# kcat/openal-soft

Hardware: NVIDIA H100
Metric: voice-samples/s mixed (HRTF, bsinc24, 1024-frame updates) (higher is better)
Workload: dtype f32

## Files before the change

openal-soft_b200/csrc/b200mix.cu:

```cuda
#include "../../include/b200mix.h"

#include <algorithm>
#include <cmath>
#include <cstdio>
#include <cstdlib>
#include <cstring>
#include <new>
#include <string>
#include <vector>

#include <cuda_runtime.h>

#include <dlfcn.h>

#include "mixer_kernels.cuh"
#include "effect_kernels.cuh"
#include "shard_kernels.cuh"
#include "panmix_tc.cuh"
#include "param_kernels.hpp"
#include "efx_kernels.hpp"
#include "resampler_tables.hpp"
#include "hrtf_store.hpp"
#include "adpcm.hpp"

// ... 145 lines not shown
    uint32_t num_order{0};
    bool order_dirty{true};

    char *h_src{nullptr}, *d_src{nullptr}; uint32_t src_cap{0};
    cudaEvent_t src_done{nullptr}; bool src_busy{false};
    bool dev_filters{false};
    bool panmix_tc{false};
    bool mix_gather_only{false};

    struct Shard {
        uint32_t rank{0}, world{1}; int transport{0};
        char *own{nullptr}; size_t bytes{0};
        char *peer[kShardMaxWorld]{};
        size_t off_real{0}, off_wet{0}, real_floats{0}, wet_src_floats{0};
        uint32_t owned_max{0};
        uint32_t epoch{0};
        uint32_t *d_counters{nullptr};
        uint32_t *h_status{nullptr};
        cudaEvent_t ev[4]{};
        bool ev_wet{false}, ev_real{false};
        void *nccl_lib{nullptr}; void *comm{nullptr};
        int (*reduce)(const void*, void*, size_t, int, int, int, void*, cudaStream_t){nullptr};
        int (*allreduce)(const void*, void*, size_t, int, int, void*, cudaStream_t){nullptr};
        int (*comm_destroy)(void*){nullptr};
    } shard;

    uint32_t ir_pad{0};
    uint32_t voice_hi{0};
    int mix_variant{0}; int mix_groups{2}; int mix_gs{64}; int mix_cdr{0};
    uint32_t reverb_seq{0};
    size_t mix_smem{0}; int mix_blocks_per_sm{1};
    uint32_t *d_claim{nullptr};
    int fir_blocks_per_sm{0};
};

namespace {

#define CUDA_TRY(dev, expr) do { cudaError_t e_ = (expr); if(e_ != cudaSuccess) {            \
    (dev)->error = std::string(#expr) + ": " + cudaGetErrorString(e_); return B200MIX_ERR_CUDA; } } while(0)

template<typename T>
int dev_alloc(b200mix_device *d, T *&p, size_t count, bool zero = true)
{
    p = nullptr;
    if(count == 0) return B200MIX_OK;
    CUDA_TRY(d, cudaMalloc(reinterpret_cast<void**>(&p), count*sizeof(T)));
    if(zero) CUDA_TRY(d, cudaMemsetAsync(p, 0, count*sizeof(T), d->stream));
    return B200MIX_OK;
}

using MixKernel = void(*)(const MixParams);

struct Variant { MixKernel fn; int gs, groups, cdr; size_t smem; };

template<int GS, int GROUPS, int CDR>
Variant make_variant()
{
    return Variant{k_mix_voices<GS, GROUPS, CDR>, GS, GROUPS, CDR, sizeof(GroupSmem<CDR>)*GROUPS};
}

Variant get_variant(int idx)
{
    return idx == 0 ? make_variant<64, 2, 4>() : make_variant<64, 2, 0>();
}

struct FirVariant { MixKernel fn; size_t smem; };
// ... 144 lines not shown
        if(int rc = dev_alloc(d, d->d_dry_cur, size_t(dd.max_voices)*std::max(dd.dry_channels, 1u))) return rc;
        if(int rc = dev_alloc(d, d->d_dry_tgt, size_t(dd.max_voices)*std::max(dd.dry_channels, 1u))) return rc;
        if(dd.num_sends && dd.wet_channels)
        {
            const size_t per = size_t(dd.num_sends)*dd.wet_channels;
            if(int rc = dev_alloc(d, d->d_send_cur, dd.max_voices*per)) return rc;
            if(int rc = dev_alloc(d, d->d_send_tgt, dd.max_voices*per)) return rc;
        }
        if(int rc = dev_alloc(d, d->d_order, dd.max_voices)) return rc;
        d->h_active.assign(dd.max_voices, 0);
        d->h_cost.assign(dd.max_voices, 0);
        d->h_hrtf.assign(dd.max_voices, 0);

        const bool hrtfDev = dd.ir_size > 0;
        d->mix_variant = (!hrtfDev && dd.dry_channels <= 4) ? 0 : 1;
        const Variant var = get_variant(d->mix_variant);
        d->mix_gs = var.gs; d->mix_groups = var.groups; d->mix_cdr = var.cdr; d->mix_smem = var.smem;
        CUDA_TRY(d, cudaFuncSetAttribute(var.fn, cudaFuncAttributeMaxDynamicSharedMemorySize, int(var.smem)));
        int perSm = 0;
        CUDA_TRY(d, cudaOccupancyMaxActiveBlocksPerMultiprocessor(&perSm, var.fn, var.gs*var.groups, var.smem));
        d->mix_blocks_per_sm = std::max(perSm, 1);
        if(var.cdr == 0)
        {
            if(int rc = dev_alloc(d, d->d_xscratch, size_t(dd.max_voices)*kLine)) return rc;
            if(int rc = dev_alloc(d, d->d_sendinfo, dd.max_voices)) return rc;
            if(int rc = dev_alloc(d, d->d_claim, 2)) return rc;
        }
        if(hrtfDev)
        {
            const FirVariant fir = get_fir(dd.ir_size);
            CUDA_TRY(d, cudaFuncSetAttribute(fir.fn, cudaFuncAttributeMaxDynamicSharedMemorySize, int(fir.smem)));
            CUDA_TRY(d, cudaOccupancyMaxActiveBlocksPerMultiprocessor(&perSm, fir.fn, kFirGS*kFirGroups, fir.smem));
            d->fir_blocks_per_sm = std::max(std::min(perSm, kFirCtasPerSm), 1);
        }

        d->dry_alloc_ch = std::max<uint32_t>(std::max(dd.dry_channels, 1u), uint32_t(var.cdr));
        if(int rc = dev_alloc(d, d->d_dry, size_t(d->dry_alloc_ch)*kLine)) return rc;
        {
            const size_t realFloats = size_t(std::max(dd.real_channels, 1u))*kLine;
            static_assert(sizeof(VoiceResult) == 16 && sizeof(b200mix_voice_result) == 16, "result layout");
            const size_t blockBytes = realFloats*sizeof(float) + size_t(dd.max_voices)*sizeof(VoiceResult);
            char *blk = nullptr;
            if(int rc = dev_alloc(d, blk, blockBytes)) return rc;
            d->d_outblock = blk;
            d->d_results = reinterpret_cast<VoiceResult*>(blk + realFloats*sizeof(float));
            CUDA_TRY(d, cudaMallocHost(reinterpret_cast<void**>(&d->h_outblock), blockBytes));
            d->h_real = reinterpret_cast<float*>(d->h_outblock);
            d->h_results = reinterpret_cast<b200mix_voice_result*>(d->h_outblock + realFloats*sizeof(float));
            d->out_real_bytes = realFloats*sizeof(float);
            if(dd.post_process == B200MIX_POST_NONE) d->d_real = d->d_dry;
            else d->d_real = reinterpret_cast<float*>(blk);
        }
        if(dd.max_slots && dd.wet_channels)
            if(int rc = dev_alloc(d, d->d_wet, size_t(dd.max_slots)*dd.wet_channels*kLine)) return rc;
        d->partial_floats = hrtfDev ? size_t(d->num_sms)*d->fir_blocks_per_sm*(2*kAccumLen)
            : size_t(d->num_sms)*d->mix_blocks_per_sm*size_t(var.cdr)*kLine;
        if(int rc = dev_alloc(d, d->d_partial, std::max<size_t>((hrtfDev ? 1 : 2)*d->partial_floats, 4))) return rc;
        if(int rc = dev_alloc(d, d->d_accum_sum, 2*kAccumLen)) return rc;
        if(int rc = dev_alloc(d, d->d_carry[0], 2*kHrirLen)) return rc;
        if(int rc = dev_alloc(d, d->d_carry[1], 2*kHrirLen)) return rc;
        if(int rc = dev_alloc(d, d->d_temp, size_t(std::max(dd.dry_channels, 1u))*kLine)) return rc;
        if(int rc = dev_alloc(d, d->d_temp2, size_t(std::max(dd.dry_channels, 1u))*kLine)) return rc;
        if(dd.max_slots && dd.wet_channels && dd.num_sends)
        {
            d->h_slots.assign(dd.max_slots, SlotRec{});
            d->slot_allocs.assign(dd.max_slots, {});
// ... 30 lines not shown
        }
        if(int rc = ensure_stage(d, std::min(dd.max_voices, 4096u))) return rc;
        CUDA_TRY(d, cudaStreamSynchronize(d->stream));
        return B200MIX_OK;
    };
    int rc;
    try { rc = run(); }
    catch(const std::exception &e) { d->error = e.what(); rc = B200MIX_ERR_NOMEM; }
    if(rc != B200MIX_OK) return fail(rc);
    *out = d;
    return B200MIX_OK;
}

void b200mix_destroy(b200mix_device *d)
{
    if(!d) return;
    if(d->stream) cudaStreamSynchronize(d->stream);
    shard_release(d);
    for(auto &b : d->h_buffers) if(b.data) cudaFree(const_cast<void*>(b.data));
    for(int i = 0;i < 3;++i) cudaFree(d->d_bsinc[i]);
    for(int i = 0;i < 2;++i) cudaFree(d->d_cubic[i]);
    cudaFree(d->d_voices); cudaFree(d->d_buffers); cudaFree(d->d_hrtf_tgt); cudaFree(d->d_hrtf_old);
    cudaFree(d->d_dry_cur); cudaFree(d->d_dry_tgt); cudaFree(d->d_send_cur); cudaFree(d->d_send_tgt);
    cudaFree(d->d_outblock); cudaFreeHost(d->h_outblock); cudaFree(d->d_order);
    cudaFree(d->d_dry); cudaFree(d->d_wet); cudaFree(d->d_partial); cudaFree(d->d_accum_sum);
    cudaFree(d->d_carry[0]); cudaFree(d->d_carry[1]);
    cudaFree(d->d_dec_coef); cudaFree(d->d_dec_hfscale); cudaFree(d->d_dec_state);
    cudaFree(d->d_temp); cudaFree(d->d_temp2);
    cudaFree(d->d_amb_hf); cudaFree(d->d_amb_lf); cudaFree(d->d_amb_state);
    cudaFree(d->d_uhj_state); cudaFree(d->d_uhj_scratch);
    cudaFree(d->d_uhj_fir_state); cudaFree(d->d_uhj_fir_coef); cudaFree(d->d_bs2b); cudaFree(d->d_stab_state);
    for(auto &v : d->slot_allocs) for(void *p : v) cudaFree(p);
    cudaFree(d->d_slots); cudaFree(d->d_xscratch); cudaFree(d->d_sendinfo); cudaFree(d->d_claim);
    cudaFree(d->d_filt); cudaFree(d->d_fupd); cudaFree(d->d_fscratch);
    cudaFree(d->d_dline); cudaFree(d->d_order2); cudaFree(d->d_qhdr); cudaFree(d->d_queue);
    cudaFree(d->d_outbuf); if(d->h_outbuf) cudaFreeHost(d->h_outbuf);
    cudaFree(d->d_limiter); cudaFree(d->d_limiter_delay);
    cudaFree(d->d_dc_delay); cudaFree(d->d_dc_gain); cudaFree(d->d_dc_buf);
    cudaFree(d->d_st_fields); cudaFree(d->d_st_elevs); cudaFree(d->d_st_coeffs); cudaFree(d->d_st_delays);
    cudaFree(d->d_dry_entries); cudaFree(d->d_dry_slot_start); cudaFree(d->d_dry_partial);
    cudaFree(d->d_dry_geff); cudaFree(d->d_send_geff); cudaFree(d->d_send_partial);
    cudaFree(d->d_dry_gramp); cudaFree(d->d_send_gramp);
    if(d->h_fupd) cudaFreeHost(d->h_fupd);
    if(d->fstage_done) cudaEventDestroy(d->fstage_done);
    cudaFree(d->d_slot_start); cudaFree(d->d_entries); cudaFree(d->d_twiddle); cudaFree(d->d_cubic_filter);
    cudaFree(d->d_efx_views);
    cudaFreeHost(d->h_arena); cudaFree(d->d_arena);
    if(d->h_src) cudaFreeHost(d->h_src);
    cudaFree(d->d_src);
    if(d->src_done) cudaEventDestroy(d->src_done);
    if(d->stage_done) cudaEventDestroy(d->stage_done);
    if(d->ev_mix0) cudaEventDestroy(d->ev_mix0);
    if(d->ev_mix1) cudaEventDestroy(d->ev_mix1);
    for(cudaEvent_t e : d->ev_stage) if(e) cudaEventDestroy(e);
    if(d->stream) cudaStreamDestroy(d->stream);
    delete d;
}

int b200mix_set_hrtf_decoder(b200mix_device *d, uint32_t channels, uint32_t ir_size,
    const float *coeffs, const float *hf_scale, const float *splitter_coeff)
{
    if(!d || channels != d->desc.dry_channels || ir_size > B200MIX_HRIR_LENGTH || !coeffs
        || !hf_scale || !splitter_coeff || d->desc.post_process != B200MIX_POST_HRTF)
    { if(d) d->error = "set_hrtf_decoder: bad arguments"; return B200MIX_ERR_INVALID; }
    CUDA_TRY(d, cudaSetDevice(d->cuda_dev));
    cudaFree(d->d_dec_coef); cudaFree(d->d_dec_hfscale); cudaFree(d->d_dec_state);
// ... 1115 lines not shown
        if(d->num_order2)
        {
            CUDA_TRY(d, cudaMemcpyAsync(d->d_order2, d->h_order2.data(), d->num_order2*sizeof(uint32_t),
                cudaMemcpyHostToDevice, d->stream));
            CUDA_TRY(d, cudaStreamSynchronize(d->stream));
        }
        d->order2_dirty = false;
    }
    const Variant var = get_variant(d->mix_variant);
    const bool hrtfDev = dd.ir_size > 0;
    const uint32_t nv = std::max(d->voice_hi, 1u);
    const uint32_t maxBlocks = uint32_t(d->num_sms*d->mix_blocks_per_sm);
    const uint32_t blocks = std::max(1u, std::min(maxBlocks, (d->num_order + var.groups - 1)/var.groups));

    MixParams P{};
    P.voices = d->d_voices; P.buffers = d->d_buffers;
    P.hrtf_tgt = d->d_hrtf_tgt; P.hrtf_old = d->d_hrtf_old;
    P.dry_cur = d->d_dry_cur; P.dry_tgt = d->d_dry_tgt;
    P.send_cur = d->d_send_cur; P.send_tgt = d->d_send_tgt;
    P.dry = d->d_dry; P.wet = d->d_wet; P.partial = d->d_partial;
    P.results = want_results ? d->d_results : nullptr;
    for(int i = 0;i < 3;++i) P.bsinc_tab[i] = d->d_bsinc[i];
    for(int i = 0;i < 2;++i) P.cubic_tab[i] = d->d_cubic[i];
    P.max_voices = nv; P.frames = frames; P.ir = dd.ir_size; P.ir_pad = d->ir_pad;
    P.cd = dd.dry_channels; P.cw = dd.wet_channels; P.num_sends = dd.num_sends;
    P.max_buffers = dd.max_buffers;
    P.order = d->d_order; P.num_order = d->num_order;
    P.xscratch = d->d_xscratch; P.sendinfo = d->d_sendinfo;
    P.filt = d->d_filt; P.filt_paths = 1u + dd.num_sends;
    P.qhdr = d->d_qhdr; P.queue = d->d_queue;
    P.gather_only = d->mix_gather_only ? 1u : 0u;
    P.claim = d->d_claim;
    P.dline = d->d_dline;
    stage_mark(d, 1);
    if(d->profile) cudaEventRecord(d->ev_mix0, d->stream);
    var.fn<<<blocks, var.gs*var.groups, var.smem, d->stream>>>(P);
    ++d->launches;
    CUDA_TRY(d, cudaGetLastError());

    stage_mark(d, 2);
    size_t rows2 = 0;
    if(d->d_filt && d->num_order2)
    {
        FilterRunParams FP{};
        FP.filt = d->d_filt; FP.filt_paths = 1u + dd.num_sends; FP.sendinfo = d->d_sendinfo;
        FP.direct_order = d->d_order2; FP.num_direct = d->num_order2;
        FP.xscratch = d->d_xscratch; FP.dline = d->d_dline; FP.frames = frames;
        k_filters<<<(d->num_order2 + 31u)/32u, 32, 0, d->stream>>>(FP);
        ++d->launches;
        if(var.cdr > 0)
        {
            const uint32_t blocks2 = std::max(1u, std::min(maxBlocks, (d->num_order2 + var.groups - 1)/var.groups));
            rows2 = blocks2;
            MixParams P2 = P;
            P2.pass = 1u;
            P2.order = d->d_order2; P2.num_order = d->num_order2;
            P2.partial = d->d_partial + d->partial_floats;
            P2.results = nullptr;
            var.fn<<<blocks2, var.gs*var.groups, var.smem, d->stream>>>(P2);
            ++d->launches;
        }
        CUDA_TRY(d, cudaGetLastError());
    }
    uint32_t firBlocks = 0;
    if(hrtfDev)
    {
        const FirVariant fir = get_fir(dd.ir_size);
        firBlocks = std::max(1u, std::min(uint32_t(d->num_sms*d->fir_blocks_per_sm),
            (d->num_order + kFirGroups - 1)/kFirGroups));
        fir.fn<<<firBlocks, kFirGS*kFirGroups, fir.smem, d->stream>>>(P);
        ++d->launches;
        CUDA_TRY(d, cudaGetLastError());
    }
    if(d->profile) { cudaEventRecord(d->ev_mix1, d->stream); d->ev_valid = true; }

    stage_mark(d, 3);
    if(hrtfDev)
    {
        const uint32_t len = 2*kAccumLen;
        k_reduce_rows<<<(len/4 + kReduceCols - 1)/kReduceCols, 1024, 0, d->stream>>>(d->d_partial, firBlocks, len,
            d->d_accum_sum, 0);
        ++d->launches;
    }
    if(var.cdr > 0)
    {
        const uint32_t len = uint32_t(var.cdr)*kLine;
        k_reduce_rows<<<(len/4 + kReduceCols - 1)/kReduceCols, 1024, 0, d->stream>>>(d->d_partial, blocks, len, d->d_dry, 1);
        ++d->launches;
        if(rows2)
        {
            k_reduce_rows<<<(len/4 + kReduceCols - 1)/kReduceCols, 1024, 0, d->stream>>>(d->d_partial + d->partial_floats,
                uint32_t(rows2), len, d->d_dry, 1);
            ++d->launches;
        }
    }
    CUDA_TRY(d, cudaGetLastError());

    stage_mark(d, 4);
    if(var.cdr == 0 && d->d_dry_entries)
    {
        if(d->dry_entries_dirty)
        {
            d->h_dry_entries.clear();
            for(uint32_t v = 0;v < d->voice_hi;++v)
                if(d->h_active[v] && !d->h_hrtf[v]) d->h_dry_entries.push_back(SendEntry{v, 0u});
            d->num_dry_entries = uint32_t(d->h_dry_entries.size());
// ... 439 lines not shown
static int render_launch(b200mix_device *d, uint32_t frames, bool want_results)
{
    if(d->mid_render) { d->error = "render: a render_begin is pending"; return B200MIX_ERR_INVALID; }
    const bool sharded = d->shard.transport != 0;
    if(sharded) ++d->shard.epoch;
    if(int rc = render_phase_a(d, frames, want_results, sharded)) return rc;
    if(sharded) if(int rc = shard_wet_exchange(d)) return rc;
    if(int rc = render_phase_b(d, frames)) return rc;
    if(sharded) if(int rc = shard_real_reduce(d)) return rc;
    return render_output_stage(d, frames);
}

static int render_collect(b200mix_device *d, uint32_t frames, float *const *real_out,
    b200mix_voice_result *results)
{
    const b200mix_device_desc &dd = d->desc;
    const uint32_t nv = std::max(d->voice_hi, 1u);
    const bool contiguous = d->d_real == reinterpret_cast<float*>(d->d_outblock);
    if(real_out && results && contiguous)
        CUDA_TRY(d, cudaMemcpyAsync(d->h_outblock, d->d_outblock, d->out_real_bytes + size_t(nv)*sizeof(VoiceResult),
            cudaMemcpyDeviceToHost, d->stream));
    else
    {
        if(real_out)
            CUDA_TRY(d, cudaMemcpyAsync(d->h_real, d->d_real, size_t(dd.real_channels)*kLine*sizeof(float),
                cudaMemcpyDeviceToHost, d->stream));
        if(results)
            CUDA_TRY(d, cudaMemcpyAsync(d->h_results, d->d_results, size_t(nv)*sizeof(VoiceResult),
                cudaMemcpyDeviceToHost, d->stream));
    }
    if(d->shard.transport == 1)
        CUDA_TRY(d, cudaMemcpyAsync(d->shard.h_status, d->shard.own + offsetof(ShardCtl, status),
            sizeof(uint32_t), cudaMemcpyDeviceToHost, d->stream));
    CUDA_TRY(d, cudaStreamSynchronize(d->stream));
    d->stage_busy = false;
    if(d->shard.transport == 1 && *d->shard.h_status)
    { d->error = "render: a peer of the sharded device set did not answer in time"; return B200MIX_ERR_CUDA; }
    if(real_out)
        for(uint32_t c = 0;c < dd.real_channels;++c)
            if(real_out[c]) std::memcpy(real_out[c], d->h_real + size_t(c)*kLine, frames*sizeof(float));
    if(results)
    {
        std::memcpy(results, d->h_results, size_t(nv)*sizeof(b200mix_voice_result));
        for(uint32_t v = nv;v < dd.max_voices;++v)
            results[v] = b200mix_voice_result{0, 0u, B200MIX_VF_STOPPED, 0u};
    }
    return B200MIX_OK;
}

int b200mix_render(b200mix_device *d, uint32_t frames, float *const *real_out,
    b200mix_voice_result *results)
{
    if(!d) return B200MIX_ERR_INVALID;
    if(int rc = render_launch(d, frames, results != nullptr)) return rc;
    return render_collect(d, frames, real_out, results);
}

int b200mix_set_uhj_encoder(b200mix_device *d, uint32_t filter_length, uint32_t *delay)
{
    if(!d) return B200MIX_ERR_INVALID;
    const b200mix_device_desc &dd = d->desc;
    if(d->mid_render || (dd.post_process != B200MIX_POST_UHJ && dd.post_process != B200MIX_POST_TSME)
        || dd.dry_channels < 3
        || (filter_length != 0 && filter_length != 256 && filter_length != 512))
    { d->error = "set_uhj_encoder: needs a UHJ device and a length of 0, 256 or 512"; return B200MIX_ERR_INVALID; }
    CUDA_TRY(d, cudaStreamSynchronize(d->stream));
    CUDA_TRY(d, cudaMemset(d->d_uhj_state, 0, 64*sizeof(float)));
    if(filter_length)
// ... 460 lines not shown
```

openal-soft_b200/csrc/mixer_kernels.cuh:

```cuda
#pragma once
#include <cstdint>
#include <cuda_runtime.h>

#include "voice_structs.hpp"
#include "async_ptx.cuh"

namespace b200mix {

constexpr int kLine = 1024;
constexpr int kHrirLen = 128;
constexpr int kHist = 64;
constexpr int kEdge = 24;
constexpr int kPad = 48;
constexpr int kResBuf = kLine + 256 + kPad;
constexpr int kSrcSizeMax = kResBuf - kEdge;
constexpr int kAccumLen = kLine + kHrirLen;
constexpr float kSilence = 0.00001f;
constexpr float kEps = 1.1920929e-07f;

constexpr uint32_t kVfStatic = 1u<<2, kVfLooping = 1u<<3, kVfHrtf = 1u<<4;
constexpr uint32_t kVfFading = 1u<<8, kVfHaveBuffer = 1u<<9, kVfCoefDirty = 1u<<10;
constexpr uint32_t kUpNoBuffer = 1u<<11;
constexpr uint32_t kVfChannelMask = 0xffu<<16;

struct alignas(16) BufferRec {
    const void *data;
    uint32_t frames, type, channels, pad;
};

struct alignas(16) VoiceRec {
    uint32_t state;
    uint32_t flags;
    uint32_t buffer, resampler;
// ... 10 lines not shown

struct alignas(16) FilterRec {
    float cur[2][5]; float tgt[2][5];
    float z[2][2];
    int32_t counter[2];
    uint32_t active;
    uint32_t pad[5];
};
static_assert(sizeof(FilterRec) == 128, "FilterRec layout");

struct MixParams {
    VoiceRec *voices; const BufferRec *buffers;
    float2 *hrtf_tgt; float2 *hrtf_old;
    float *dry_cur; float *dry_tgt;
    float *send_cur; float *send_tgt;
    float *dry;
    float *wet;
    float *partial;
    VoiceResult *results;
    const float *bsinc_tab[3];
    const float *cubic_tab[2];
    uint32_t max_voices, frames, ir, ir_pad, cd, cw, num_sends, max_buffers;
    float *xscratch;
    uint32_t *sendinfo;
    const uint32_t *order;
    uint32_t num_order;
    FilterRec *filt;
    uint32_t filt_paths;
    uint32_t pass;
    const float *dline;
    uint4 *qhdr; const uint32_t *queue;
    uint32_t gather_only;
    uint32_t *claim;
};

constexpr uint32_t kMaxQueue = 32, kNoLoop = 0xffffffffu;

constexpr uint32_t kSiSend = 1u, kSiPlaying = 2u, kSiDeferred = 4u, kSiDirty = 8u, kSiDry = 16u,
    kSiHrtf = 32u;

__device__ __forceinline__ void group_sync(int id, int count)
{
    if(id == 1) asm volatile("bar.sync 1, %0;" :: "r"(count) : "memory");
    else asm volatile("bar.sync 2, %0;" :: "r"(count) : "memory");
}

__device__ __forceinline__ void prefetch_l2(const void *p)
{ asm volatile("prefetch.global.L2 [%0];" :: "l"(p)); }

__device__ __forceinline__ uint32_t sample_bytes(uint32_t type)
{ return type == 1u ? 2u : ((type == 0u || type >= 5u) ? 1u : (type == 4u ? 8u : 4u)); }

__device__ __forceinline__ void prefetch_span(const char *base, size_t bytes, size_t off,
    size_t len, int t, int gs)
{
    if(off >= bytes) return;
    if(off + len > bytes) len = bytes - off;
    const size_t first = off & ~size_t(127);
    for(size_t a = first + size_t(t)*128u;a < off + len;a += size_t(gs)*128u)
        prefetch_l2(base + a);
}

__device__ __forceinline__ float load_sample(const BufferRec &b, size_t idx)
{
    switch(b.type)
    {
// ... 88 lines not shown
            k = k < A.count ? k : A.count-1u;
            uint32_t q;
            if(!A.looping) q = min(A.uintPos + k, A.lastFrame);
            else if(k < A.firstRun) q = A.q0 + k;
            else if(A.simpleWrap) q = A.loopStart + (k - A.firstRun);
            else q = A.loopStart + (k - A.firstRun)%A.loopSize;
            raw[u] = ld_raw(src + size_t(q)*A.channels);
        }
        #pragma unroll
        for(int u = 0;u < 8;++u)
        {
            const uint32_t k = k0 + uint32_t(u)*GS;
            if(k < A.count) A.dst[k] = A.pastEnd ? 0.0f : to_float(raw[u]);
        }
    }
}

template<int CDR>
struct alignas(16) GroupSmem {
    static constexpr int kTabStride = kPad + 2;
    float win[kResBuf + 8 + 24];
    alignas(8) float tabF[32*kTabStride];
    alignas(8) float tabD[32*kTabStride];
    float x[CDR > 0 ? kLine : 1];
    float newGain[32];
    uint64_t tmaBar;
    uint32_t claimed;
};

template<int GS, int OPT, int FP>
struct alignas(16) FirSmem {
    static constexpr int kLLen = FP + OPT*GS;
    static constexpr int kOLen = FP + kHist + FP + 32;
    float2 lLR[kLLen];
    float2 oLR[kOLen];
    float x[kHist + kLine];
    float2 coefT[kHrirLen], coefO[kHrirLen];
};

__device__ __forceinline__ float2 fma2_rn(float2 a, float2 b, float2 c)
{ return make_float2(__fmaf_rn(a.x, b.x, c.x), __fmaf_rn(a.y, b.y, c.y)); }

template<int OPT, int FP>
__device__ __forceinline__ void fir_pass(float2 (&acc)[OPT], const float2 *__restrict__ in,
    const float2 *__restrict__ coef, int irpad, int t0)
{
    constexpr int JB = 8;
    for(int jb = 0;jb < irpad;jb += JB)
    {
        float2 w[OPT+JB-1];
        const float2 *p = in + FP + t0 - jb - (JB-1);
        #pragma unroll
        for(int k = 0;k < OPT+JB-1;++k) w[k] = p[k];
        #pragma unroll
        for(int jj = 0;jj < JB;++jj)
        {
            const float2 c = coef[jb+jj];
            #pragma unroll
            for(int r = 0;r < OPT;++r)
                acc[r] = fma2_rn(c, w[r - jj + (JB-1)], acc[r]);
        }
    }
}

__device__ __forceinline__ uint32_t claim_voice(const MixParams &P, uint32_t &slot, int t, int bar,
    int gs, uint32_t groups)
{
    group_sync(bar, gs);
    if(t == 0)
    {
        uint32_t oi = atomicAdd(P.claim, 1u);
        if(oi >= P.num_order && atomicAdd(P.claim + 1, 1u) == groups - 1u)
        {
            atomicExch(P.claim, 0u);
            atomicExch(P.claim + 1, 0u);
        }
        slot = oi;
    }
    group_sync(bar, gs);
    return slot;
}

template<int GS, int GROUPS, int CDR>
__global__ void __launch_bounds__(GS*GROUPS, GS*GROUPS != 128 ? 1 : (CDR == 0 ? 5 : 3))
k_mix_voices(const MixParams P)
{
    using Smem = GroupSmem<CDR>;
    extern __shared__ __align__(16) unsigned char smem_raw[];
    const int g = threadIdx.x / GS;
    const int t = threadIdx.x % GS;
    Smem &S = reinterpret_cast<Smem*>(smem_raw)[g];
    const int bar = 1 + g;
    constexpr int SPT = kLine / GS;

    float accD[CDR > 0 ? CDR : 1][SPT];
    #pragma unroll
    for(int c = 0;c < (CDR > 0 ? CDR : 1);++c)
        #pragma unroll
        for(int r = 0;r < SPT;++r) accD[c][r] = 0.0f;

    const uint32_t n = P.frames;
    if(t == 0) { mbar_init(&S.tmaBar, 1u); mbar_fence_init(); }
    uint32_t tmaPhase = 0u;
    group_sync(bar, GS);

    const uint32_t groups = gridDim.x*GROUPS;
    for(uint32_t oi = CDR > 0 ? blockIdx.x*GROUPS + g : claim_voice(P, S.claimed, t, bar, GS, groups);
        oi < P.num_order;
        oi = CDR > 0 ? oi + groups : claim_voice(P, S.claimed, t, bar, GS, groups))
    {
        const uint32_t v = P.order[oi];
        VoiceRec &rec = P.voices[v];
        const uint4 *hp = reinterpret_cast<const uint4*>(&rec);
        const uint4 h0 = hp[0], h1 = hp[1], h2 = hp[2], h3 = hp[3], h4 = hp[4];
        const bool second = P.pass != 0u;
        uint32_t info = 0u;
        if(second)
        {
            info = P.sendinfo[v];
            if(!(info & kSiDeferred)) continue;
        }
        const uint32_t vstate = second ? ((info & kSiPlaying) ? 1u : 2u) : h0.x;
        if(vstate != 1u && vstate != 2u)
        {
            if(t == 0)
            {
                if(P.results) P.results[v] = VoiceResult{int32_t(h1.x), h1.y, 1u<<7, 0u};
                if(P.sendinfo) P.sendinfo[v] = 0u;
            }
            continue;
        }
        const uint32_t increment = h1.z;
        uint32_t flags = h0.y;
        if(!second && increment < 1u)
        {
// ... 542 lines not shown
        float *stage = reinterpret_cast<float*>(smem_raw);
        float *pd = P.partial + row*(size_t(CDR)*kLine);
        if(GROUPS == 1)
        {
            #pragma unroll
            for(int c = 0;c < (CDR > 0 ? CDR : 1);++c)
                #pragma unroll
                for(int r = 0;r < SPT;++r)
                    pd[c*kLine + t + r*GS] = accD[c][r];
        }
        else
        {
            for(int gg = 0;gg < GROUPS;++gg)
            {
                if(g == gg)
                {
                    #pragma unroll
                    for(int c = 0;c < (CDR > 0 ? CDR : 1);++c)
                        #pragma unroll
                        for(int r = 0;r < SPT;++r)
                        {
                            float *dst = stage + c*kLine + t + r*GS;
                            if(gg == 0) *dst = accD[c][r]; else *dst += accD[c][r];
                        }
                }
                __syncthreads();
            }
            for(int o = threadIdx.x;o < CDR*kLine;o += GS*GROUPS) pd[o] = stage[o];
        }
    }
}

constexpr int kFirGS = 64, kFirGroups = 2, kFirCtasPerSm = 4;

template<int OPT, int FP>
__global__ void __launch_bounds__(kFirGS*kFirGroups, kFirCtasPerSm)
k_hrtf_fir(const MixParams P)
{
    constexpr int GS = kFirGS, GROUPS = kFirGroups;
    using Smem = FirSmem<GS, OPT, FP>;
    extern __shared__ __align__(16) unsigned char smem_raw[];
    const int g = threadIdx.x / GS;
    const int t = threadIdx.x % GS;
    Smem &S = reinterpret_cast<Smem*>(smem_raw)[g];
    const int bar = 1 + g;
    const int t0 = OPT*t;
    const uint32_t n = P.frames;

    float2 acc[OPT];
    #pragma unroll
    for(int r = 0;r < OPT;++r) acc[r] = make_float2(0.0f, 0.0f);

    const uint32_t stride = gridDim.x*GROUPS;
    for(uint32_t oi = blockIdx.x*GROUPS + g;oi < P.num_order;oi += stride)
    {
        const uint32_t v = P.order[oi];
        const uint32_t info = P.sendinfo[v];
        if(!(info & kSiHrtf)) continue;
        VoiceRec &rec = P.voices[v];
        const uint4 *hp = reinterpret_cast<const uint4*>(&rec);
        const uint4 h3 = hp[3], h4 = hp[4];
        const bool playing = (info & kSiPlaying) != 0;
        const bool dirty = (info & kSiDirty) != 0;
        const uint32_t counter = (info >> 8) & 0xffu;

        const float *line = ((info & kSiDeferred) ? P.dline : P.xscratch) + size_t(v)*kLine;
        for(int k = t;k < kHist;k += GS) S.x[k] = rec.hist[k];
        for(uint32_t k = t;k < n;k += GS) S.x[kHist + k] = line[k];
        const float2 *ct = P.hrtf_tgt + size_t(v)*P.ir_pad;
        const float2 *co = P.hrtf_old + size_t(v)*P.ir_pad;
        for(int k = t;k < int(P.ir_pad);k += GS)
        {
            const float2 c = ct[k];
            S.coefT[k] = c;
            S.coefO[k] = dirty ? co[k] : c;
        }
        group_sync(bar, GS);


        if(playing)
            for(int k = t;k < kHist;k += GS) rec.hist[k] = S.x[n + k];
        uint32_t oD0 = h4.x, oD1 = h4.y;
        float oGain = __uint_as_float(h4.z);
        const uint32_t tD0 = h3.y, tD1 = h3.z;
        const float tgtGain = __uint_as_float(h3.w);
        if(!counter) { oD0 = tD0; oD1 = tD1; oGain = tgtGain; }
        const bool sameFilter = !counter || (!dirty && oD0 == tD0 && oD1 == tD1);
        const float targetGain = tgtGain * (playing ? 1.0f : 0.0f);
        const uint32_t fademix = counter;
        float blendNewStep = 0.0f, oldStep = 0.0f;
        bool oldOn = false, newOn = false;
        float gainA = oGain;
        if(fademix)
        {
            const float gain = targetGain;
            blendNewStep = gain / float(fademix);
            oldStep = oGain / float(fademix);
            oldOn = oGain > kSilence;
            newOn = blendNewStep*float(fademix) > kSilence;
            gainA = gain;
        }
        const uint32_t todo = n - fademix;
        const float step2 = todo ? (targetGain - gainA) / float(todo) : 0.0f;

        const float *hs = S.x;
        for(int i = t;i < Smem::kLLen;i += GS)
        {
            const int s = i - FP;
            float l = 0.0f, r = 0.0f;
            if(s >= 0 && s < int(n))
            {
                float gnew;
                if(uint32_t(s) < fademix)
                    gnew = (newOn && s >= 1) ? blendNewStep*float(s) : 0.0f;
                else
                    gnew = gainA + step2*float(uint32_t(s) - fademix);
                l = hs[kHist - tD0 + s] * gnew;
                r = hs[kHist - tD1 + s] * gnew;
                if(sameFilter && oldOn && uint32_t(s) < fademix)
                {
                    const float gold = oldStep*float(fademix - uint32_t(s));
                    l += hs[kHist - oD0 + s] * gold;
                    r += hs[kHist - oD1 + s] * gold;
                }
            }
            S.lLR[i] = make_float2(l, r);
        }
        const bool oldPass = !sameFilter && oldOn;
        if(oldPass)
            for(int i = t;i < Smem::kOLen;i += GS)
            {
                const int s = i - FP;
                float l = 0.0f, r = 0.0f;
                if(s >= 0 && uint32_t(s) < fademix)
                {
                    const float gold = oldStep*float(fademix - uint32_t(s));
                    l = hs[kHist - oD0 + s] * gold;
                    r = hs[kHist - oD1 + s] * gold;
                }
                S.oLR[i] = make_float2(l, r);
            }
        group_sync(bar, GS);

        {
            const uint32_t o2 = oi + 2u*stride, o1 = oi + stride;
            const uint32_t v2 = o2 < P.num_order ? P.order[o2] : 0xffffffffu;
            const uint32_t v1 = o1 < P.num_order ? P.order[o1] : 0xffffffffu;
            if(v2 < P.max_voices)
            {
                if(t < 5) prefetch_l2(reinterpret_cast<const char*>(&P.voices[v2]) + t*128);
                else if(t < 5 + int((P.ir_pad*8u + 127u)/128u))
                    prefetch_l2(reinterpret_cast<const char*>(P.hrtf_tgt + size_t(v2)*P.ir_pad) + (t-5)*128);
            }
            if(v1 < P.max_voices && t < int(kLine*sizeof(float)/128u))
            {
                const float *nl = ((P.sendinfo[v1] & kSiDeferred) ? P.dline : P.xscratch) + size_t(v1)*kLine;
                prefetch_l2(reinterpret_cast<const char*>(nl) + t*128);
            }
        }

        const int irpad = int(P.ir_pad);
        fir_pass<OPT, FP>(acc, S.lLR, S.coefT, irpad, t0);
        if(oldPass && t0 < int(kHist) + irpad)
            fir_pass<OPT, FP>(acc, S.oLR, S.coefO, irpad, t0);
        if(t == 0)
        {
            rec.old_delay0 = tD0; rec.old_delay1 = tD1;
            rec.old_gain = targetGain;
        }
        group_sync(bar, GS);
    }

    const size_t row = blockIdx.x;
    __syncthreads();
    float *stage = reinterpret_cast<float*>(smem_raw);
    for(int gg = 0;gg < GROUPS;++gg)
    {
        if(g == gg)
        {
            #pragma unroll
            for(int r = 0;r < OPT;++r)
            {
                const int o = t0 + r;
                if(o < kAccumLen)
                {
                    if(gg == 0) { stage[o] = acc[r].x; stage[kAccumLen + o] = acc[r].y; }
                    else { stage[o] += acc[r].x; stage[kAccumLen + o] += acc[r].y; }
                }
            }
            if(gg == 0 && GS*OPT < kAccumLen)
                for(int o = GS*OPT + t;o < kAccumLen;o += GS) { stage[o] = 0.0f; stage[kAccumLen + o] = 0.0f; }
        }
        __syncthreads();
    }
    float *pl = P.partial + row*(2*kAccumLen);
    for(int o = threadIdx.x;o < 2*kAccumLen;o += GS*GROUPS) pl[o] = stage[o];
}


constexpr int kReduceCols = 8, kReduceSegs = 128;
__global__ void __launch_bounds__(1024)
k_reduce_rows(const float *__restrict__ partial, uint32_t rows, uint32_t len,
    float *__restrict__ out, int accumulate)
{
    __shared__ float4 sm[kReduceSegs][kReduceCols];
    const uint32_t col = threadIdx.x & (kReduceCols-1), seg = threadIdx.x / kReduceCols;
    const uint32_t e4 = blockIdx.x*kReduceCols + col;
    float4 s = make_float4(0.f, 0.f, 0.f, 0.f);
    if(e4*4u < len)
    {
        const uint32_t per = (rows + kReduceSegs - 1u)/kReduceSegs;
        const uint32_t r0 = seg*per, r1 = (r0 + per < rows) ? r0 + per : rows;
        const float4 *p = reinterpret_cast<const float4*>(partial) + e4;
        const size_t stride4 = len/4u;
        uint32_t r = r0;
        for(;r + 4u <= r1;r += 4u)
        {
            const float4 a = __ldg(p + size_t(r)*stride4), b = __ldg(p + size_t(r+1)*stride4);
            const float4 c = __ldg(p + size_t(r+2)*stride4), d = __ldg(p + size_t(r+3)*stride4);
            s.x += a.x; s.y += a.y; s.z += a.z; s.w += a.w;
            s.x += b.x; s.y += b.y; s.z += b.z; s.w += b.w;
            s.x += c.x; s.y += c.y; s.z += c.z; s.w += c.w;
            s.x += d.x; s.y += d.y; s.z += d.z; s.w += d.w;
        }
        for(;r < r1;++r)
        {
            const float4 a = __ldg(p + size_t(r)*stride4);
            s.x += a.x; s.y += a.y; s.z += a.z; s.w += a.w;
        }
// ... 1117 lines not shown
```

Baseline: 28.07 billion.

## Overlap HRTF FIR kernel with mixer tail via programmatic dependent launch

Launches the HRIR FIR kernel with programmatic stream serialization so it can start while the mixer kernel's last voices are still being resampled. Per-voice ready flags (epoch-tagged, release/acquire) and a tail counter let FIR groups wait only for voices in the mixer's tail, and the mixer triggers dependents once a group claims a tail slot. This aims to hide the launch gap and the mixer's tail imbalance, at the cost of spin-waiting with a timeout, extra global atomics, and a new error path reported to the host.

```diff
diff --git a/openal-soft_b200/csrc/b200mix.cu b/openal-soft_b200/csrc/b200mix.cu
--- a/openal-soft_b200/csrc/b200mix.cu
+++ b/openal-soft_b200/csrc/b200mix.cu
@@ -201,6 +201,8 @@
     size_t mix_smem{0}; int mix_blocks_per_sm{1};
     uint32_t *d_claim{nullptr};
     int fir_blocks_per_sm{0};
+    uint32_t *d_ready{nullptr}; uint32_t fir_epoch{0};
+    uint32_t *d_fir_sync{nullptr}; uint32_t fir_tail_target{0}; uint32_t *h_fir_status{nullptr};
 };
 
 namespace {
@@ -411,6 +413,10 @@
             CUDA_TRY(d, cudaFuncSetAttribute(fir.fn, cudaFuncAttributeMaxDynamicSharedMemorySize, int(fir.smem)));
             CUDA_TRY(d, cudaOccupancyMaxActiveBlocksPerMultiprocessor(&perSm, fir.fn, kFirGS*kFirGroups, fir.smem));
             d->fir_blocks_per_sm = std::max(std::min(perSm, kFirCtasPerSm), 1);
+            if(int rc = dev_alloc(d, d->d_ready, dd.max_voices)) return rc;
+            if(int rc = dev_alloc(d, d->d_fir_sync, 2)) return rc;
+            CUDA_TRY(d, cudaMallocHost(reinterpret_cast<void**>(&d->h_fir_status), sizeof(uint32_t)));
+            *d->h_fir_status = 0u;
         }
 
         d->dry_alloc_ch = std::max<uint32_t>(std::max(dd.dry_channels, 1u), uint32_t(var.cdr));
@@ -507,6 +513,8 @@
     cudaFree(d->d_uhj_fir_state); cudaFree(d->d_uhj_fir_coef); cudaFree(d->d_bs2b); cudaFree(d->d_stab_state);
     for(auto &v : d->slot_allocs) for(void *p : v) cudaFree(p);
     cudaFree(d->d_slots); cudaFree(d->d_xscratch); cudaFree(d->d_sendinfo); cudaFree(d->d_claim);
+    cudaFree(d->d_ready); cudaFree(d->d_fir_sync);
+    if(d->h_fir_status) cudaFreeHost(d->h_fir_status);
     cudaFree(d->d_filt); cudaFree(d->d_fupd); cudaFree(d->d_fscratch);
     cudaFree(d->d_dline); cudaFree(d->d_order2); cudaFree(d->d_qhdr); cudaFree(d->d_queue);
     cudaFree(d->d_outbuf); if(d->h_outbuf) cudaFreeHost(d->h_outbuf);
@@ -1688,13 +1696,23 @@
     P.gather_only = d->mix_gather_only ? 1u : 0u;
     P.claim = d->d_claim;
     P.dline = d->d_dline;
+    const bool firEarly = hrtfDev && !(d->d_filt && d->num_order2);
+    if(firEarly)
+    {
+        if(++d->fir_epoch == 0u) d->fir_epoch = 1u;
+        const uint32_t groups = blocks*uint32_t(var.groups);
+        d->fir_tail_target += groups;
+        P.ready = d->d_ready; P.fir_sync = d->d_fir_sync; P.epoch = d->fir_epoch;
+        P.tail_start = d->num_order > groups ? d->num_order - groups : 0u;
+        P.tail_target = d->fir_tail_target;
+    }
     stage_mark(d, 1);
     if(d->profile) cudaEventRecord(d->ev_mix0, d->stream);
     var.fn<<<blocks, var.gs*var.groups, var.smem, d->stream>>>(P);
     ++d->launches;
     CUDA_TRY(d, cudaGetLastError());
 
-    stage_mark(d, 2);
+    if(!firEarly) stage_mark(d, 2);
     size_t rows2 = 0;
     if(d->d_filt && d->num_order2)
     {
@@ -1724,10 +1742,17 @@
         const FirVariant fir = get_fir(dd.ir_size);
         firBlocks = std::max(1u, std::min(uint32_t(d->num_sms*d->fir_blocks_per_sm),
             (d->num_order + kFirGroups - 1)/kFirGroups));
-        fir.fn<<<firBlocks, kFirGS*kFirGroups, fir.smem, d->stream>>>(P);
+        cudaLaunchConfig_t cfg{};
+        cfg.gridDim = dim3(firBlocks); cfg.blockDim = dim3(kFirGS*kFirGroups);
+        cfg.dynamicSmemBytes = fir.smem; cfg.stream = d->stream;
+        cudaLaunchAttribute attr{};
+        attr.id = cudaLaunchAttributeProgrammaticStreamSerialization;
+        attr.val.programmaticStreamSerializationAllowed = 1;
+        if(firEarly) { cfg.attrs = &attr; cfg.numAttrs = 1; }
+        CUDA_TRY(d, cudaLaunchKernelEx(&cfg, fir.fn, P));
         ++d->launches;
-        CUDA_TRY(d, cudaGetLastError());
-    }
+    }
+    if(firEarly) stage_mark(d, 2);
     if(d->profile) { cudaEventRecord(d->ev_mix1, d->stream); d->ev_valid = true; }
 
     stage_mark(d, 3);
@@ -2233,8 +2258,13 @@
     if(d->shard.transport == 1)
         CUDA_TRY(d, cudaMemcpyAsync(d->shard.h_status, d->shard.own + offsetof(ShardCtl, status),
             sizeof(uint32_t), cudaMemcpyDeviceToHost, d->stream));
+    if(d->d_fir_sync)
+        CUDA_TRY(d, cudaMemcpyAsync(d->h_fir_status, d->d_fir_sync, sizeof(uint32_t),
+            cudaMemcpyDeviceToHost, d->stream));
     CUDA_TRY(d, cudaStreamSynchronize(d->stream));
     d->stage_busy = false;
+    if(d->d_fir_sync && *d->h_fir_status)
+    { d->error = "render: the HRIR FIR kernel timed out waiting for a resampled voice"; return B200MIX_ERR_CUDA; }
     if(d->shard.transport == 1 && *d->shard.h_status)
     { d->error = "render: a peer of the sharded device set did not answer in time"; return B200MIX_ERR_CUDA; }
     if(real_out)
diff --git a/openal-soft_b200/csrc/mixer_kernels.cuh b/openal-soft_b200/csrc/mixer_kernels.cuh
--- a/openal-soft_b200/csrc/mixer_kernels.cuh
+++ b/openal-soft_b200/csrc/mixer_kernels.cuh
@@ -75,6 +75,7 @@
     uint4 *qhdr; const uint32_t *queue;
     uint32_t gather_only;
     uint32_t *claim;
+    uint32_t *ready; uint32_t *fir_sync; uint32_t epoch, tail_start, tail_target;
 };
 
 constexpr uint32_t kMaxQueue = 32, kNoLoop = 0xffffffffu;
@@ -260,21 +261,41 @@
     }
 }
 
+__device__ __forceinline__ uint32_t ld_relaxed_gpu(const uint32_t *p)
+{
+    uint32_t v;
+    asm volatile("ld.relaxed.gpu.global.u32 %0, [%1];" : "=r"(v) : "l"(p) : "memory");
+    return v;
+}
+__device__ __forceinline__ uint32_t ld_acquire_gpu(const uint32_t *p)
+{
+    uint32_t v;
+    asm volatile("ld.acquire.gpu.global.u32 %0, [%1];" : "=r"(v) : "l"(p) : "memory");
+    return v;
+}
+__device__ __forceinline__ void st_release_gpu(uint32_t *p, uint32_t v)
+{ asm volatile("st.release.gpu.global.u32 [%0], %1;" :: "l"(p), "r"(v) : "memory"); }
+
 __device__ __forceinline__ uint32_t claim_voice(const MixParams &P, uint32_t &slot, int t, int bar,
     int gs, uint32_t groups)
 {
     group_sync(bar, gs);
     if(t == 0)
     {
+        if(P.ready && slot >= P.tail_start && slot < P.num_order)
+            st_release_gpu(P.ready + P.order[slot], P.epoch);
         uint32_t oi = atomicAdd(P.claim, 1u);
         if(oi >= P.num_order && atomicAdd(P.claim + 1, 1u) == groups - 1u)
         {
             atomicExch(P.claim, 0u);
             atomicExch(P.claim + 1, 0u);
         }
+        if(P.ready && oi >= P.tail_start && (slot == ~0u || slot < P.tail_start))
+            asm volatile("red.release.gpu.global.add.u32 [%0], 1;" :: "l"(P.fir_sync + 1) : "memory");
         slot = oi;
     }
     group_sync(bar, gs);
+    if(P.ready && slot >= P.tail_start) asm volatile("griddepcontrol.launch_dependents;" ::: "memory");
     return slot;
 }
 
@@ -297,7 +318,7 @@
         for(int r = 0;r < SPT;++r) accD[c][r] = 0.0f;
 
     const uint32_t n = P.frames;
-    if(t == 0) { mbar_init(&S.tmaBar, 1u); mbar_fence_init(); }
+    if(t == 0) { mbar_init(&S.tmaBar, 1u); mbar_fence_init(); S.claimed = ~0u; }
     uint32_t tmaPhase = 0u;
     group_sync(bar, GS);
 
@@ -906,6 +927,23 @@
 }
 
 constexpr int kFirGS = 64, kFirGroups = 2, kFirCtasPerSm = 4;
+constexpr unsigned long long kFirWaitTimeoutNs = 4000000000ull;
+
+__device__ __forceinline__ bool wait_published(const uint32_t *flag, uint32_t value, uint32_t *status)
+{
+    if(int32_t(ld_relaxed_gpu(flag) - value) < 0)
+    {
+        unsigned long long t0, t1;
+        asm volatile("mov.u64 %0, %%globaltimer;" : "=l"(t0));
+        while(int32_t(ld_relaxed_gpu(flag) - value) < 0)
+        {
+            asm volatile("mov.u64 %0, %%globaltimer;" : "=l"(t1));
+            if(t1 - t0 > kFirWaitTimeoutNs) { atomicExch(status, 1u); return false; }
+            __nanosleep(128);
+        }
+    }
+    return int32_t(ld_acquire_gpu(flag) - value) >= 0;
+}
 
 template<int OPT, int FP>
 __global__ void __launch_bounds__(kFirGS*kFirGroups, kFirCtasPerSm)
@@ -926,10 +964,21 @@
     for(int r = 0;r < OPT;++r) acc[r] = make_float2(0.0f, 0.0f);
 
     const uint32_t stride = gridDim.x*GROUPS;
+    bool waiting = true;
+    if(P.ready)
+    {
+        if(t == 0) waiting = wait_published(P.fir_sync + 1, P.tail_target, P.fir_sync);
+        group_sync(bar, GS);
+    }
     for(uint32_t oi = blockIdx.x*GROUPS + g;oi < P.num_order;oi += stride)
     {
         const uint32_t v = P.order[oi];
-        const uint32_t info = P.sendinfo[v];
+        if(P.ready && oi >= P.tail_start)
+        {
+            if(t == 0 && waiting) waiting = wait_published(P.ready + v, P.epoch, P.fir_sync);
+            group_sync(bar, GS);
+        }
+        const uint32_t info = __ldcg(P.sendinfo + v);
         if(!(info & kSiHrtf)) continue;
         VoiceRec &rec = P.voices[v];
         const uint4 *hp = reinterpret_cast<const uint4*>(&rec);
@@ -940,7 +989,7 @@
 
         const float *line = ((info & kSiDeferred) ? P.dline : P.xscratch) + size_t(v)*kLine;
         for(int k = t;k < kHist;k += GS) S.x[k] = rec.hist[k];
-        for(uint32_t k = t;k < n;k += GS) S.x[kHist + k] = line[k];
+        for(uint32_t k = t;k < n;k += GS) S.x[kHist + k] = __ldcg(line + k);
         const float2 *ct = P.hrtf_tgt + size_t(v)*P.ir_pad;
         const float2 *co = P.hrtf_old + size_t(v)*P.ir_pad;
         for(int k = t;k < int(P.ir_pad);k += GS)
@@ -1069,6 +1118,7 @@
     }
     float *pl = P.partial + row*(2*kAccumLen);
     for(int o = threadIdx.x;o < 2*kAccumLen;o += GS*GROUPS) pl[o] = stage[o];
+    if(P.ready) asm volatile("griddepcontrol.wait;" ::: "memory");
 }
 
 
```

Result: faster. 28.50 billion, median of 6 (+1.5%).

## Double-buffer HRTF FIR voice staging with TMA bulk copies and mbarriers

Applied to the files above, without the earlier changes.

Replaces the per-voice thread-strided global-to-shared loads of history, input line, coefficients and voice header with bulk async copies issued by one thread into a two-slot shared staging buffer guarded by mbarriers. The next voice is staged while the current one is filtered, which hides load latency and drops the explicit input-line L2 prefetch. In exchange the shared memory footprint per group roughly doubles for the staged data, which can lower occupancy against the four-CTA launch bound. Correctness now depends on mbarrier parity tracking and on buffer reuse being ordered with the end-of-iteration group sync.

```diff
diff --git a/openal-soft_b200/csrc/mixer_kernels.cuh b/openal-soft_b200/csrc/mixer_kernels.cuh
--- a/openal-soft_b200/csrc/mixer_kernels.cuh
+++ b/openal-soft_b200/csrc/mixer_kernels.cuh
@@ -1,4 +1,5 @@
 #pragma once
+#include <cstddef>
 #include <cstdint>
 #include <cuda_runtime.h>
 
@@ -229,10 +230,16 @@
 struct alignas(16) FirSmem {
     static constexpr int kLLen = FP + OPT*GS;
     static constexpr int kOLen = FP + kHist + FP + 32;
+    struct alignas(16) Stage {
+        float x[kHist + kLine];
+        float2 coefT[kHrirLen], coefO[kHrirLen];
+        uint4 h34[2];
+    };
     float2 lLR[kLLen];
     float2 oLR[kOLen];
-    float x[kHist + kLine];
-    float2 coefT[kHrirLen], coefO[kHrirLen];
+    Stage st[2];
+    uint64_t bar[2];
+    uint32_t oi[2], v[2], info[2];
 };
 
 __device__ __forceinline__ float2 fma2_rn(float2 a, float2 b, float2 c)
@@ -907,12 +914,43 @@
 
 constexpr int kFirGS = 64, kFirGroups = 2, kFirCtasPerSm = 4;
 
+template<class Smem>
+__device__ __forceinline__ void fir_stage_voice(const MixParams &P, Smem &S, uint32_t oi,
+    uint32_t stride, int b)
+{
+    uint32_t v = 0u, info = 0u;
+    for(;oi < P.num_order;oi += stride)
+    {
+        v = P.order[oi];
+        info = P.sendinfo[v];
+        if(info & kSiHrtf) break;
+    }
+    S.oi[b] = oi; S.v[b] = v; S.info[b] = info;
+    if(oi >= P.num_order) return;
+    typename Smem::Stage &st = S.st[b];
+    const VoiceRec &rec = P.voices[v];
+    const float *line = ((info & kSiDeferred) ? P.dline : P.xscratch) + size_t(v)*kLine;
+    const bool dirty = (info & kSiDirty) != 0;
+    const uint32_t lineBytes = (P.frames*4u + 15u) & ~15u;
+    const uint32_t hrBytes = P.ir_pad*uint32_t(sizeof(float2));
+    fence_proxy_async_smem();
+    mbar_expect_tx(&S.bar[b], uint32_t(sizeof(rec.hist)) + lineBytes + uint32_t(sizeof(st.h34))
+        + (dirty ? 2u : 1u)*hrBytes);
+    bulk_g2s(st.x, rec.hist, uint32_t(sizeof(rec.hist)), &S.bar[b]);
+    if(lineBytes) bulk_g2s(st.x + kHist, line, lineBytes, &S.bar[b]);
+    bulk_g2s(st.h34, reinterpret_cast<const uint4*>(&rec) + 3, uint32_t(sizeof(st.h34)), &S.bar[b]);
+    bulk_g2s(st.coefT, P.hrtf_tgt + size_t(v)*P.ir_pad, hrBytes, &S.bar[b]);
+    if(dirty) bulk_g2s(st.coefO, P.hrtf_old + size_t(v)*P.ir_pad, hrBytes, &S.bar[b]);
+}
+
 template<int OPT, int FP>
 __global__ void __launch_bounds__(kFirGS*kFirGroups, kFirCtasPerSm)
 k_hrtf_fir(const MixParams P)
 {
     constexpr int GS = kFirGS, GROUPS = kFirGroups;
     using Smem = FirSmem<GS, OPT, FP>;
+    static_assert(sizeof(VoiceRec::hist) % 16 == 0 && offsetof(VoiceRec, hist) % 16 == 0,
+        "History is bulk-copied");
     extern __shared__ __align__(16) unsigned char smem_raw[];
     const int g = threadIdx.x / GS;
     const int t = threadIdx.x % GS;
@@ -926,34 +964,29 @@
     for(int r = 0;r < OPT;++r) acc[r] = make_float2(0.0f, 0.0f);
 
     const uint32_t stride = gridDim.x*GROUPS;
-    for(uint32_t oi = blockIdx.x*GROUPS + g;oi < P.num_order;oi += stride)
-    {
-        const uint32_t v = P.order[oi];
-        const uint32_t info = P.sendinfo[v];
-        if(!(info & kSiHrtf)) continue;
+    if(t == 0)
+    {
+        mbar_init(&S.bar[0], 1u); mbar_init(&S.bar[1], 1u); mbar_fence_init();
+        fir_stage_voice(P, S, blockIdx.x*GROUPS + g, stride, 0);
+    }
+    group_sync(bar, GS);
+    uint32_t parity = 0u;
+    for(int cur = 0;S.oi[cur] < P.num_order;cur ^= 1)
+    {
+        const uint32_t oi = S.oi[cur], v = S.v[cur], info = S.info[cur];
+        if(t == 0) fir_stage_voice(P, S, oi + stride, stride, cur ^ 1);
         VoiceRec &rec = P.voices[v];
-        const uint4 *hp = reinterpret_cast<const uint4*>(&rec);
-        const uint4 h3 = hp[3], h4 = hp[4];
         const bool playing = (info & kSiPlaying) != 0;
         const bool dirty = (info & kSiDirty) != 0;
         const uint32_t counter = (info >> 8) & 0xffu;
-
-        const float *line = ((info & kSiDeferred) ? P.dline : P.xscratch) + size_t(v)*kLine;
-        for(int k = t;k < kHist;k += GS) S.x[k] = rec.hist[k];
-        for(uint32_t k = t;k < n;k += GS) S.x[kHist + k] = line[k];
-        const float2 *ct = P.hrtf_tgt + size_t(v)*P.ir_pad;
-        const float2 *co = P.hrtf_old + size_t(v)*P.ir_pad;
-        for(int k = t;k < int(P.ir_pad);k += GS)
-        {
-            const float2 c = ct[k];
-            S.coefT[k] = c;
-            S.coefO[k] = dirty ? co[k] : c;
-        }
-        group_sync(bar, GS);
-
+        typename Smem::Stage &st = S.st[cur];
+        mbar_wait(&S.bar[cur], (parity >> cur) & 1u);
+        parity ^= 1u << cur;
+        const uint4 h3 = st.h34[0], h4 = st.h34[1];
+        const float2 *coefO = dirty ? st.coefO : st.coefT;
 
         if(playing)
-            for(int k = t;k < kHist;k += GS) rec.hist[k] = S.x[n + k];
+            for(int k = t;k < kHist;k += GS) rec.hist[k] = st.x[n + k];
         uint32_t oD0 = h4.x, oD1 = h4.y;
         float oGain = __uint_as_float(h4.z);
         const uint32_t tD0 = h3.y, tD1 = h3.z;
@@ -977,7 +1010,7 @@
         const uint32_t todo = n - fademix;
         const float step2 = todo ? (targetGain - gainA) / float(todo) : 0.0f;
 
-        const float *hs = S.x;
+        const float *hs = st.x;
         for(int i = t;i < Smem::kLLen;i += GS)
         {
             const int s = i - FP;
@@ -1017,26 +1050,20 @@
         group_sync(bar, GS);
 
         {
-            const uint32_t o2 = oi + 2u*stride, o1 = oi + stride;
+            const uint32_t o2 = oi + 2u*stride;
             const uint32_t v2 = o2 < P.num_order ? P.order[o2] : 0xffffffffu;
-            const uint32_t v1 = o1 < P.num_order ? P.order[o1] : 0xffffffffu;
             if(v2 < P.max_voices)
             {
                 if(t < 5) prefetch_l2(reinterpret_cast<const char*>(&P.voices[v2]) + t*128);
                 else if(t < 5 + int((P.ir_pad*8u + 127u)/128u))
                     prefetch_l2(reinterpret_cast<const char*>(P.hrtf_tgt + size_t(v2)*P.ir_pad) + (t-5)*128);
             }
-            if(v1 < P.max_voices && t < int(kLine*sizeof(float)/128u))
-            {
-                const float *nl = ((P.sendinfo[v1] & kSiDeferred) ? P.dline : P.xscratch) + size_t(v1)*kLine;
-                prefetch_l2(reinterpret_cast<const char*>(nl) + t*128);
-            }
         }
 
         const int irpad = int(P.ir_pad);
-        fir_pass<OPT, FP>(acc, S.lLR, S.coefT, irpad, t0);
+        fir_pass<OPT, FP>(acc, S.lLR, st.coefT, irpad, t0);
         if(oldPass && t0 < int(kHist) + irpad)
-            fir_pass<OPT, FP>(acc, S.oLR, S.coefO, irpad, t0);
+            fir_pass<OPT, FP>(acc, S.oLR, coefO, irpad, t0);
         if(t == 0)
         {
             rec.old_delay0 = tD0; rec.old_delay1 = tD1;
```

Result: faster. 28.19 billion before, 29.04 billion after (median of 6 runs) (+3.0%).
